# DiltheyLab/HLA-LA

Hardware: AMD Instinct MI355X
Metric: paired reads/sec aligned to PRG graph (higher is better)
Workload: dtype int32

## Files before the change

hla-la_amd/csrc/batch.h:

```cpp
#pragma once
#include "device_common.h"

namespace hlala {

template <template <class> class Ptr> struct DevBatchT {
    int n_pairs, n_reads, n_chains, stride;
    int from_seeds;
    int unpaired;
    Ptr<const int> read_off;
    Ptr<const uint8_t> read_bases;
    Ptr<const uint8_t> read_quals;
    Ptr<const int> chain_off;
    Ptr<const int> read_primary;
    Ptr<const int> chain_read;
    Ptr<const int> chain_contig;
    Ptr<const int> chain_pos;
    Ptr<const int> chain_offset;
    Ptr<const int> chain_as;
    Ptr<const uint8_t> chain_reverse;
    Ptr<const int> cigar_off;
    Ptr<const u32> cigar;
    Ptr<int> seed_status;
    Ptr<int> seed_ncols;
    Ptr<int> seed_begin;
// ... 20 lines not shown
    Ptr<int> ext_edge;
    Ptr<uint8_t> ext_g;
    Ptr<uint8_t> ext_s;
    Ptr<uint8_t> ext_fromseed;
    Ptr<int> ext_firstlast;
    Ptr<int> pair_status;
    Ptr<int> best_chain;
    Ptr<int> n_comb;
    Ptr<double> pair_ll;
    Ptr<double> pair_mapq;
    Ptr<double> mate_mapq;
    Ptr<uint8_t> strands_valid;
    Ptr<uint8_t> sel_mapq;
    Ptr<u64> counters;
    Ptr<int> work_counter;
    Ptr<int> retry_list;
    Ptr<int> pair_multi;
    Ptr<uint8_t> pair_deferred;
    Ptr<int> chain_order;
    Ptr<int> chain_bucket;
    Ptr<int> order_hist;
    int order_shift, order_nb;
    int long_chunk_nodes, long_max_segs;
    int order_cost;
    Ptr<int> chain_row;
    int n_rows;
    Ptr<int> dp_blk;
    Ptr<int> dp_list;
    int dp_nblk;
    int dp_band;
    int dp_band_risky;
    int dp_jf;
    int dp_long;
    Ptr<void> dp_items;
    Ptr<int> dbg;
};
typedef DevBatchT<HostP> DevBatch;
typedef DevBatchT<GlobP> DevBatchG;
static_assert(sizeof(DevBatch) == sizeof(DevBatchG), "one layout");
__device__ __forceinline__ const DevBatchG& dev_view(const DevBatch* p) { return *(const DevBatchG*)p; }
enum { DESC_VALUE = 0, DESC_VIEW = 1, DESC_GENERIC = 2 };
template <int FORM, class D> __device__ __forceinline__ decltype(auto) desc_of(const D& byValue, const D* inMemory)
{
    if constexpr (FORM == DESC_VIEW) return dev_view(inMemory);
    else if constexpr (FORM == DESC_GENERIC) return (*inMemory);
    else return (byValue);
}

template <class BT> __device__ __forceinline__ int ordered_chains(const BT& B) { return B.chain_order ? __builtin_amdgcn_readfirstlane(B.order_hist[B.order_nb - 1]) : B.n_chains; }

template <class BT> __device__ __forceinline__ size_t row_base(const BT& B, int c) { return (size_t)(B.chain_row ? B.chain_row[c] : c) * (size_t)B.stride; }

enum { DPL_BAND16 = 0, DPL_BAND32 = 2, DPL_BAND64 = 4, DPL_JF = 6, DPL_GEN = 10, DPL_N = 14 };
__host__ __device__ inline int dpl_list(int cls, int dir, bool isLong)
{
    if(cls >= 2) return (cls == 2 ? DPL_BAND16 : (cls == 3 ? DPL_BAND32 : DPL_BAND64)) + dir;
    return (cls == 1 ? DPL_JF : DPL_GEN) + 2 * dir + (isLong ? 0 : 1);
}
__host__ __device__ inline int dp_bases_left(int dir, int seqLen, int start_seq) { return dir ? seqLen - start_seq : start_seq; }
__host__ __device__ inline bool dp_is_long(int dpLong, int dir, int seqLen, int start_seq) { return dpLong > 0 && dp_bases_left(dir, seqLen, start_seq) >= dpLong; }
enum { WC_PAIR_MULTI = 40, WC_PAIR_OVER = 72, WC_BAND_FETCH = 48, WC_FO_COUNT = 54, WC_FO_FETCH = 56, WC_BAND_FAILED = 58, WC_BAND_CALLS = 59, WC_JF_FAILED = 60, WC_BAND_WHY = 62, WC_BAND_TIED = 68,
       WC_RETRY_LONG = 88, WC_N = 100 };
__host__ __device__ inline int wc_retry_short(int tier, int dir) { return 12 + 4 * (tier - 1) + 2 * dir; }
__host__ __device__ inline int wc_retry_fetch(int tier, int dir) { return 13 + 4 * (tier - 1) + 2 * dir; }
__host__ __device__ inline int wc_retry_long(int tier, int dir) { return WC_RETRY_LONG + 2 * (tier - 1) + dir; }
__host__ __device__ inline int retry_entry(int w, int nLong, int nChains) { return w < nLong ? w : nChains - 1 - (w - nLong); }
constexpr int BAND_MAXJ16 = 15, BAND_MAXJ32 = 31, BAND_MAXJ64 = 48;

enum {
    CNT_CHAINS_EXT = 0, CNT_DP_CALLS, CNT_DP_ITERS, CNT_DP_CELLS, CNT_SEED_COLS, CNT_OUT_COLS, CNT_EDGES, CNT_ERRORS, CNT_DP_SHARED
};

}
```

hla-la_amd/csrc/hlala_api.hip:

```cpp
#include <cmath>
#include <cstdio>
#include <cstring>
#include <cstdlib>
#include <algorithm>
#include <map>
#include <mutex>
#include <chrono>
#include <thread>
#include <set>
#include <string>
#include <unordered_map>
#include <vector>

#include "../../include/hlala_gpu.h"
#include "batch.h"
#include "flat_graph.hpp"
#include "host_internal.h"

#include "kernel_dp.hip"
#include "kernel_project.hip"
#include "kernel_order.hip"
#include "kernel_pair.hip"
#include "kernel_pair_overflow.hip"
#include "kernel_typer.hip"
// ... 19 lines not shown
    void* p = nullptr; size_t bytes = 0;
};

struct DpClass {
    int grid = 0, block = 0;
    char* slabs = nullptr; size_t slab_bytes = 0;
    const char* name = "";
    void (*launch)(hlala_ctx* c, const DpClass& k, hipStream_t ws, hlala_batch* b, const DpPoolArgs& pool) = nullptr;
};

struct hlala_ctx {
    int device = 0;
    hipStream_t stream = nullptr;
    hipStream_t side = nullptr;
    hipStream_t up = nullptr, rs = nullptr, active = nullptr;
    int tail_pool_k = 1; std::vector<hlala_batch*> tail;
    hipEvent_t evSideTail = nullptr; bool sideTailValid = false;
    hlala_params params{};
    FlatGraph F;
    DevGraph G{};
    DevGraph* dG = nullptr;
    DevTables* dT = nullptr;
    double* d_islog = nullptr;
    long long* d_contig_off = nullptr; uint8_t* d_contig_seq = nullptr; int* d_contig_level = nullptr;
    int n_contigs = 0; std::vector<long long> contig_off;
    std::vector<void*> allocs;
    std::unordered_map<void*, size_t> block_bytes;
    std::multimap<size_t, void*> pool;
    size_t pool_bytes = 0;
    size_t pool_cap = (size_t)176 << 30;
    std::mutex pool_mu;
    std::set<struct hlala_batch*> batches;
    int dp_long_bases = 48;
    int jf_margin = 16;
    int stitch_by_row = 1;
    int stitch_draw = 12;
    bool side_after_pair = false;
    bool rows_all = false;
    bool band_risky = false;
    int band_grid = 0, band_margin = 8;
    DpClass dp[DP_LAST_TIER + 1]; DpClass dp_jf;
    int stitch_grid = 0;
    char* proj_slabs = nullptr; size_t proj_slab_bytes = 0; int proj_grid = 0, pair_grid = 0, pair_lean_grid = 0;
    char* rethread_slabs = nullptr; size_t rethread_slab_bytes = 0; int rethread_grid = 0;
    double* pair_scratch = nullptr;
    char* pair_over_slabs = nullptr; long long pair_over_scratch = 0, pair_over_slab_bytes = 0;
    char* proj_long_slabs = nullptr; size_t proj_long_slab_bytes = 0;
    void* create_scratch = nullptr; size_t create_scratch_bytes = 0; bool create_scratch_pinned = false;
    int long_chunk_nodes = 1 << 20, long_max_segs = 1 << 20;
    int order_cost = 0;
    int order_shift = 8, order_nb = 0;
    int* dbg_host = nullptr;
    int* d_cov = nullptr; int n_cov = 0; int* d_gene_first = nullptr; int* d_gene_last = nullptr; int n_genes = 0;
    struct KeptReads { uint8_t* store = nullptr; long long* start = nullptr; int* length = nullptr; int n = 0; };
    std::vector<KeptReads> kept;
    std::string err;
};

enum BatchEvent {
    EV_PROJECT_BEGIN, EV_PROJECT_END, EV_EXTEND_BEGIN, EV_EXTEND_END, EV_PAIR_BEGIN, EV_PAIR_END,
    EV_DP_BAND_BEGIN, EV_DP_BAND_END,
    EV_DP_BEGIN, EV_DP_CLASS0_END, EV_DP_CLASS2_END, EV_DP_END,
    EV_DP_JUMP_FREE_END,
    EV_DP_CLASS_BEGIN,
    EV_DP_CLASS_END = EV_DP_CLASS_BEGIN + DP_LAST_TIER + 1,
    EV_SIDE_FORK = EV_DP_CLASS_END + DP_LAST_TIER + 1,
// ... 310 lines not shown
        rc = dev_upload(c, c->allocs, lo.data(), lo.size(), (long long**)&G.lp_off); if(rc) return fail(rc);
    }
    UPG(gap_stretch, F.gap_stretch); UPG(lp_seqid, F.lp_seqid); UPG(lp_pos, F.lp_pos);
#undef UPG
    if(contigs && contigs->n_contigs > 0) {
        c->n_contigs = contigs->n_contigs;
        c->contig_off.assign(contigs->contig_off, contigs->contig_off + contigs->n_contigs + 1);
        size_t total = (size_t)c->contig_off.back();
        std::vector<long long> co(c->contig_off.begin(), c->contig_off.end());
        rc = dev_upload(c, c->allocs, co.data(), co.size(), &c->d_contig_off); if(rc) return fail(rc);
        rc = dev_upload(c, c->allocs, contigs->contig_seq, total, &c->d_contig_seq); if(rc) return fail(rc);
        rc = dev_upload(c, c->allocs, contigs->contig_level, total, &c->d_contig_level); if(rc) return fail(rc);
    }
    rc = build_tables(c); if(rc) return fail(rc);
    rc = dev_upload(c, c->allocs, &c->G, 1, &c->dG); if(rc) return fail(rc);
    hipDeviceProp_t prop;
    if(hipGetDeviceProperties(&prop, device) != hipSuccess) { c->err = "hipGetDeviceProperties failed"; return fail(HLALA_E_DEVICE); }
    int cus = prop.multiProcessorCount > 0 ? prop.multiProcessorCount : 256;
    auto slab_pool = [&](char** out, size_t bytes, const char* what) -> int {
        if(device_malloc_retry(c->device, nullptr, (void**)out, bytes) != hipSuccess) { c->err = std::string("hipMalloc(") + what + ") failed"; return HLALA_E_DEVICE; }
        c->allocs.push_back(*out);
        if(hipMemsetAsync(*out, 0, bytes, c->active) != hipSuccess) { c->err = std::string("hipMemset(") + what + ") failed"; return HLALA_E_DEVICE; }
        return 0;
    };
    c->band_grid = cus * 20;
    if(const char* e = getenv("HLALA_DP_BAND")) { if(atoi(e) == 0) c->band_grid = 0; }
    if(const char* e = getenv("HLALA_DP_BAND_RISKY")) c->band_risky = atoi(e) != 0;
    if(const char* e = getenv("HLALA_ROWS_ALL")) c->rows_all = atoi(e) != 0;
    if(const char* e = getenv("HLALA_SIDE_AFTER_PAIR")) c->side_after_pair = atoi(e) != 0;
    if(const char* e = getenv("HLALA_POOL_CAP_GB")) { const long g = atol(e); if(g >= 0 && g <= 1024) c->pool_cap = (size_t)g << 30; }
    if(const char* e = getenv("HLALA_DP_BAND_MARGIN")) { const int m = atoi(e); if(m >= 0 && m <= 24) c->band_margin = m; }
    if(const char* e = getenv("HLALA_DP_JF_MARGIN")) { const int m = atoi(e); if(m >= 0 && m <= 200) c->jf_margin = m; }
    if(const char* e = getenv("HLALA_DP_LONG_BASES")) { const int m = atoi(e); if(m >= 0 && m <= 4096) c->dp_long_bases = m; }
    c->stitch_grid = cus * 20;
    if(const char* e = getenv("HLALA_STITCH_BY_ROW")) c->stitch_by_row = atoi(e) != 0;
    const size_t extBytes = std::max(dp_slab_bytes<DpSmall>(), dp_slab_bytes<DpWide>()), largeBytes = std::max(dp_slab_bytes<DpLarge>(), dp_slab_bytes<DpBroad>());
    DpClass* const dp = c->dp;
    c->dp_jf = dp_class<DpTinyJF, 0>(cus * 4 * DpTinyJF::WAVES, dp_slab_bytes<DpTiny>(), "k_dp<DpTinyJF>");
    dp[0] = dp_class<DpTiny, 0>(cus * 4 * DpTiny::WAVES, dp_slab_bytes<DpTiny>(), "k_dp<DpTiny>");
    dp[1] = dp_class<DpMid, 1>(cus * 16, dp_slab_bytes<DpMid>(), "k_dp<DpMid>");
    dp[2] = dp_class<DpSmall, 2>(cus * 20, extBytes, "k_dp<DpSmall>");
    dp[3] = dp_class<DpWide, 3>(cus * 7, extBytes, "k_dp<DpWide>");
    dp[4] = dp_class<DpBroad, 4>(cus * 3, largeBytes, "k_dp<DpBroad>");
    dp[5] = dp_class<DpLarge, 5>(cus, largeBytes, "k_dp<DpLarge>");
    dp[6] = dp_class<DpHuge, 6>(cus / 4 > 0 ? cus / 4 : 1, dp_inmemory_bytes<DpHuge>(), "k_dp<DpHuge>");
    if((rc = slab_pool(&dp[0].slabs, dp[0].slab_bytes * (size_t)(64 / DpTiny::GW) * (size_t)std::max(dp[0].grid, c->dp_jf.grid), "16-lane DP slabs"))) return fail(rc);
    c->dp_jf.slabs = dp[0].slabs;
    if((rc = slab_pool(&dp[1].slabs, dp[1].slab_bytes * (size_t)(64 / DpMid::GW) * (size_t)dp[1].grid, "32-lane DP slabs"))) return fail(rc);
    if((rc = slab_pool(&dp[2].slabs, extBytes * (size_t)dp[2].grid, "64-lane DP slabs"))) return fail(rc);
    if((rc = slab_pool(&dp[3].slabs, extBytes * (size_t)dp[3].grid, "wide-class DP slabs"))) return fail(rc);
    if((rc = slab_pool(&dp[4].slabs, largeBytes * (size_t)(dp[4].grid + dp[5].grid), "large-class DP slabs"))) return fail(rc);
    dp[5].slabs = dp[4].slabs + largeBytes * (size_t)dp[4].grid;
    if((rc = slab_pool(&dp[6].slabs, dp[6].slab_bytes * (size_t)dp[6].grid, "in-memory DP class"))) return fail(rc);
    c->proj_grid = cus * (c->params.max_columns <= PROJ_CAP_SHORT ? 12 : 8); c->pair_grid = cus * 16; c->pair_lean_grid = cus * 24;
    { int rcp = dev_alloc(c, c->allocs, (size_t)2 * c->pair_grid * PAIR_COMB, &c->pair_scratch, false); if(rcp) return fail(rcp); }
    if(c->params.max_columns > PROJ_CAP) {
        c->proj_grid = cus * 20;
        c->proj_long_slab_bytes = proj_long_slab_bytes();
        c->stitch_draw = 1;
        if(device_malloc_retry(c->device, nullptr, (void**)&c->proj_long_slabs, c->proj_long_slab_bytes * (size_t)c->proj_grid) != hipSuccess) { c->err = "hipMalloc(long-read projection slabs) failed"; return fail(HLALA_E_DEVICE); }
        c->allocs.push_back(c->proj_long_slabs);
    }
    c->proj_slab_bytes = proj_slab_bytes_host(c->params.max_columns, F.max_nodes_per_level);
    if(device_malloc_retry(c->device, nullptr, (void**)&c->proj_slabs, c->proj_slab_bytes * (size_t)c->proj_grid) != hipSuccess) { c->err = "hipMalloc(projection slabs) failed"; return fail(HLALA_E_DEVICE); }
    c->allocs.push_back(c->proj_slabs);
    if(!c->proj_long_slabs) {
// ... 74 lines not shown
}
int hlala_graph_get_gap_stretch(const hlala_ctx* c, uint8_t* in_stretch)
{
    if(!c || !in_stretch) return HLALA_E_ARG;
    memcpy(in_stretch, c->F.gap_stretch.data(), c->F.gap_stretch.size());
    return HLALA_OK;
}


static int batch_alloc_outputs(hlala_ctx* c, hlala_batch* b)
{
    DevBatch& B = b->B;
    size_t nc = (size_t)B.n_chains, nr = (size_t)B.n_reads, np = (size_t)B.n_pairs;
    if(!b->prepared) { B.n_rows = B.n_chains; B.chain_row = nullptr; }
    size_t rowsAlloc = (size_t)(B.n_rows > 0 ? B.n_rows : 1);
    if(b->prepared && nc >= 4096) { const size_t gran = nc / 64; rowsAlloc = (rowsAlloc + gran - 1) / gran * gran; if(rowsAlloc > nc) rowsAlloc = nc; }
    const size_t cs = rowsAlloc * (size_t)B.stride;
    int rc = 0;
#define AL(field, n, zero) do { rc = dev_alloc(c, b->allocs, (n), &B.field, zero); if(rc) return rc; } while(0)
    if(!b->prepared) { AL(seed_status, nc, true); AL(seed_ncols, nc, true); }
    AL(seed_begin, nc, true); AL(seed_end, nc, true); AL(seed_removed, nc, true);
    AL(seed_level, cs, false); AL(seed_edge, cs, false); AL(seed_g, cs, false); AL(seed_s, cs, false);
    AL(ext_status, nc, true); AL(ext_ncols, nc, true); AL(ext_begin, nc, true); AL(ext_end, nc, true); AL(ext_ll, nc, true);
    AL(dp_iters, 2 * nc, true); AL(dp_score, 2 * nc, true); AL(dp_ncols, 2 * nc, true); AL(dp_sb, 2 * nc, true); AL(dp_se, 2 * nc, true); AL(dp_err, 2 * nc, true);
    AL(dp_alias_head, 2 * nc, false); AL(dp_alias_next, 2 * nc, false);
    AL(ext_level, cs, false); AL(ext_edge, cs, false); AL(ext_g, cs, false); AL(ext_s, cs, false); AL(ext_fromseed, cs, false);
    AL(ext_firstlast, 4 * nc, true);
    AL(pair_status, np, true); AL(best_chain, nr, true); AL(n_comb, np, true); AL(pair_ll, np, true); AL(pair_mapq, np, true);
    AL(mate_mapq, nr, true); AL(strands_valid, np, true); AL(sel_mapq, nr * (size_t)B.stride, true);
    AL(pair_deferred, np, true); AL(pair_multi, 7 * np, false); AL(counters, 32, true); AL(work_counter, WC_N, true); AL(retry_list, 16 * nc, false);
    { DpItem* it = nullptr; rc = dev_alloc(c, b->allocs, 2 * nc, &it, false); if(rc) return rc; B.dp_items = it; }
    B.dp_nblk = (int)((nc + 255) / 256); if(B.dp_nblk < 1) B.dp_nblk = 1;
    B.dp_jf = c->jf_margin + 1; B.dp_long = c->dp_long_bases;
    B.dp_band = c->band_grid > 0 ? c->band_margin + 1 : 0;
    B.dp_band_risky = c->band_risky ? 1 : 0;
    AL(dp_blk, (size_t)DPL_N * B.dp_nblk + 1, false); AL(dp_list, 2 * nc, false);
    if(!b->prepared) {
        B.chain_order = nullptr; B.chain_bucket = nullptr; B.order_hist = nullptr; B.order_shift = c->order_shift; B.order_nb = c->order_nb; B.order_cost = c->order_cost; B.long_chunk_nodes = c->long_chunk_nodes; B.long_max_segs = c->long_max_segs;
        if(c->order_nb > 0 && !B.from_seeds && nc > 0) { AL(chain_order, nc, false); AL(chain_bucket, nc, false); AL(order_hist, (size_t)c->order_nb + 1, false); }
    }
    B.dbg = c->dbg_host;
#undef AL
    return 0;
}

static int batch_create_impl(hlala_ctx* c, const hlala_batch_in* in, hlala_batch** out, bool unpaired);
int hlala_batch_create(hlala_ctx* c, const hlala_batch_in* in, hlala_batch** out) { return batch_create_impl(c, in, out, false); }
int hlala_batch_create_unpaired(hlala_ctx* c, const hlala_batch_in* in, hlala_batch** out) { return batch_create_impl(c, in, out, true); }

static int batch_create_impl(hlala_ctx* c, const hlala_batch_in* in, hlala_batch** out, bool unpaired)
{
    DEV_GUARD(c);
    if(!c || !in || !out) return HLALA_E_ARG;
    UploadScope upscope_(c);
    *out = nullptr;
    if(in->n_pairs < 0 || in->n_chains < 0) { c->err = "negative batch sizes"; return HLALA_E_ARG; }
    if(!c->d_contig_off) { c->err = "hlala_batch_create needs contigs (hlala_create was called without them)"; return HLALA_E_STATE; }
    static const bool hostTiming = getenv("HLALA_HOST_TIMING") != nullptr;
    const auto tc0 = std::chrono::steady_clock::now(); auto tc1 = tc0, tc2 = tc0;
    hlala_batch* b = new hlala_batch(); b->ctx = c; c->batches.insert(b);
    DevBatch& B = b->B;
    B.n_pairs = in->n_pairs; B.n_reads = (unpaired ? 1 : 2) * in->n_pairs; B.n_chains = in->n_chains; B.stride = c->params.max_columns; B.from_seeds = 0; B.unpaired = unpaired ? 1 : 0;
    int nr = B.n_reads, nc = B.n_chains;
    auto fail = [&](int rc) { (void)hipStreamSynchronize(c->active); hlala_batch_destroy(b); return rc; };
    const int64_t rb0 = nr > 0 ? in->read_off[0] : 0, cb0 = nr > 0 ? in->chain_off[0] : 0;
    if(nr > 0) {
// ... 279 lines not shown
    return check_launch(c, "k_dp_lists");
}
static int dp_band(hlala_ctx* c, hlala_batch* b)
{
    DevBatch& B = b->B;
    b->band_used = c->band_grid > 0;
    if(!b->band_used) return HLALA_OK;
    const DpItem* items = (const DpItem*)B.dp_items; const u32 seed = c->params.rng_seed + 2u * b->first_chain;
    HIP_TRY(c, hipEventRecord(b->ev[EV_DP_BAND_BEGIN], c->active));
    hipLaunchKernelGGL((k_dp_band<16>), dim3(c->band_grid), dim3(64), 0, c->active, c->G, b->B, items, seed, (const uint8_t*)B.read_bases, c->G.lin_label, c->G.lin_eid);
    hipLaunchKernelGGL((k_dp_band<32>), dim3(c->band_grid), dim3(64), 0, c->active, c->G, b->B, items, seed, (const uint8_t*)B.read_bases, c->G.lin_label, c->G.lin_eid);
    hipLaunchKernelGGL((k_dp_band<64>), dim3(c->band_grid), dim3(64), 0, c->active, c->G, b->B, items, seed, (const uint8_t*)B.read_bases, c->G.lin_label, c->G.lin_eid);
    STEP(check_launch(c, "k_dp_band"));
    HIP_TRY(c, hipEventRecord(b->ev[EV_DP_BAND_END], c->active)); return HLALA_OK;
}
static int dp_classes(hlala_ctx* c, hlala_batch* const* bs, int n, int first, int last, hipStream_t ws)
{
    const DpPoolArgs noPool{};
    DpPoolArgs pool{}; pool.n = n; hlala_batch* b0 = bs[0];
    for(int i = 0; i < n; i++) { const hlala_batch* b = bs[i]; pool.seed[i] = c->params.rng_seed + 2u * b->first_chain; pool.B[i] = b->dB; pool.items[i] = (const DpItem*)b->B.dp_items; pool.bases[i] = (const uint8_t*)b->B.read_bases; }
    for(int tier = first; tier <= last; tier++) {
        const DpClass& k = c->dp[tier];
        if(tier == 0) HIP_TRY(c, hipEventRecord(b0->ev[EV_DP_BEGIN], c->active));
        for(int i = 0; i < n; i++) HIP_TRY(c, hipEventRecord(bs[i]->ev[EV_DP_CLASS_BEGIN + tier], ws));
        if(tier == 0) {
            c->dp_jf.launch(c, c->dp_jf, ws, b0, noPool);
            STEP(check_launch(c, c->dp_jf.name));
            HIP_TRY(c, hipEventRecord(b0->ev[EV_DP_JUMP_FREE_END], ws));
        }
        k.launch(c, k, ws, b0, tier < DP_POOL_TIER ? noPool : pool);
        STEP(check_launch(c, k.name));
        for(int i = 0; i < n; i++) HIP_TRY(c, hipEventRecord(bs[i]->ev[EV_DP_CLASS_END + tier], ws));
        if(tier == 0 || tier == 2) HIP_TRY(c, hipEventRecord(b0->ev[tier == 0 ? EV_DP_CLASS0_END : EV_DP_CLASS2_END], c->active));
    }
    return HLALA_OK;
}
static int side_fork(hlala_ctx* c, hlala_batch* b)
{
    HIP_TRY(c, hipEventRecord(b->ev[EV_SIDE_FORK], c->active)); HIP_TRY(c, hipStreamWaitEvent(c->side, b->ev[EV_SIDE_FORK], 0));
    HIP_TRY(c, hipEventRecord(b->ev[EV_SIDE_BEGIN], c->side)); b->side_used = true;
    return HLALA_OK;
}
static int side_mark(hlala_ctx* c, hlala_batch* b)
{
    HIP_TRY(c, hipEventRecord(b->ev[EV_DONE], c->side)); b->side_inflight = true;
    HIP_TRY(c, hipEventRecord(c->evSideTail, c->side)); c->sideTailValid = true;
    return HLALA_OK;
}
static int stitch_main(hlala_ctx* c, hlala_batch* b, int mode)
{
    const int sgrid = b->B.n_chains < c->stitch_grid ? b->B.n_chains : c->stitch_grid;
    hipLaunchKernelGGL(k_stitch_chains, dim3(sgrid), dim3(64), 0, c->active, c->G, c->dT, b->B, (const uint8_t*)b->B.pair_deferred, mode, c->stitch_draw, c->stitch_by_row);
    return check_launch(c, "k_stitch_chains");
}
static int stitch_side(hlala_ctx* c, hlala_batch* b)
{
    const int pgrid = (b->B.n_pairs + 63) / 64, cap = c->stitch_grid / 20;
    hipLaunchKernelGGL(k_stitch_chains, dim3(pgrid < cap ? (pgrid > 0 ? pgrid : 1) : cap), dim3(64), 0, c->side, c->G, c->dT, b->B, (const uint8_t*)b->B.pair_deferred, 2, 0, 0);
    return check_launch(c, "k_stitch_chains (side)");
}
static int extend_end(hlala_ctx* c, hlala_batch* b) { HIP_TRY(c, hipEventRecord(b->ev[EV_EXTEND_END], c->active)); b->staged |= 2; return mark_main(c, b); }
static int pair_begin(hlala_ctx* c, hlala_batch* b) { HIP_TRY(c, hipMemsetAsync(b->B.work_counter + 2, 0, sizeof(int), c->active)); HIP_TRY(c, hipEventRecord(b->ev[EV_PAIR_BEGIN], c->active)); return HLALA_OK; }
static int pair_pass(hlala_ctx* c, hlala_batch* b, hipStream_t st, int mode)
{
    DevBatch& B = b->B;
    const int grid = B.n_pairs < c->pair_grid ? B.n_pairs : c->pair_grid, lean = B.n_pairs < c->pair_lean_grid ? B.n_pairs : c->pair_lean_grid;
// ... 570 lines not shown
    for(int i = 0; i < n; i++) { hlala_ctx* c = m->ctxs[(size_t)i]; DevGuard g(c->device);
        if(!c->d_cov) { c->n_cov = (int)nl; int rc = dev_alloc(c, c->allocs, nl, &c->d_cov, true); if(rc) { m->err = c->err; return rc; } }
        if(hipStreamSynchronize(c->rs) != hipSuccess || hipStreamSynchronize(c->stream) != hipSuccess) { m->err = "hlala_reduce_coverage: a context's stream failed"; return HLALA_E_DEVICE; } }
    ncclResult_t r = g_rccl.GroupStart();
    for(int i = 0; i < n && r == ncclSuccess; i++) r = g_rccl.Reduce(m->ctxs[(size_t)i]->d_cov, i == 0 ? (void*)m->covAcc : nullptr, nl, ncclInt32, ncclSum, 0, m->comms[(size_t)i], m->streams[(size_t)i]);
    const ncclResult_t re = g_rccl.GroupEnd();
    if(r == ncclSuccess) r = re;
    if(r != ncclSuccess) { m->err = std::string("RCCL reduce: ") + g_rccl.GetErrorString(r); return HLALA_E_DEVICE; }
    for(int i = 0; i < n; i++) { hlala_ctx* c = m->ctxs[(size_t)i]; DevGuard g(c->device);
        if(hipStreamSynchronize(m->streams[(size_t)i]) != hipSuccess) { m->err = "RCCL reduce: stream failed"; return HLALA_E_DEVICE; }
        if(reset && hipMemset(c->d_cov, 0, nl * sizeof(int)) != hipSuccess) { m->err = "hipMemset failed"; return HLALA_E_DEVICE; } }
    DevGuard g0(c0->device);
    if(hipMemcpy(bases_per_level, m->covAcc, nl * sizeof(int), hipMemcpyDeviceToHost) != hipSuccess) { m->err = "coverage: copy to the host failed"; return HLALA_E_DEVICE; }
    return HLALA_OK;
}


int hlala_batch_get_stats(hlala_ctx* c, hlala_batch* b, hlala_batch_stats* out)
{
    DEV_GUARD(c);
    ReaderScope rscope_(c, b); if(rscope_.rc) return rscope_.rc;
    if(!c || !b || !out) return HLALA_E_ARG;
    memset(out, 0, sizeof(*out));
    if(!b->outputs_ready) return HLALA_OK;
    HIP_TRY(c, hipStreamSynchronize(c->active));
    u64 cnt[16];
    HIP_TRY(c, hipMemcpyAsync(cnt, b->B.counters, sizeof(cnt), hipMemcpyDeviceToHost, c->active)); HIP_TRY(c, hipStreamSynchronize(c->active));
    if((b->staged & 1) && !b->B.from_seeds) (void)hipEventElapsedTime(&out->ms_project, b->ev[EV_PROJECT_BEGIN], b->ev[EV_PROJECT_END]);
    if(b->staged & 2) { (void)hipEventElapsedTime(&out->ms_extend, b->ev[EV_EXTEND_BEGIN], b->ev[EV_EXTEND_END]); if(b->B.n_chains > 0) { (void)hipEventElapsedTime(&out->ms_extend_retry, b->ev[EV_DP_CLASS0_END], b->ev[b->side_used ? EV_DP_CLASS2_END : EV_DP_END]); (void)hipEventElapsedTime(&out->ms_dp_main, b->ev[EV_DP_BEGIN], b->ev[EV_DP_CLASS0_END]);
          for(int k = 0; k <= DP_LAST_TIER; k++) (void)hipEventElapsedTime(&out->ms_dp_class[k], b->ev[EV_DP_CLASS_BEGIN + k], b->ev[EV_DP_CLASS_END + k]);
          (void)hipEventElapsedTime(&out->ms_dp_jump_free, b->ev[EV_DP_CLASS_BEGIN], b->ev[EV_DP_JUMP_FREE_END]);
          if(b->band_used) (void)hipEventElapsedTime(&out->ms_dp_band, b->ev[EV_DP_BAND_BEGIN], b->ev[EV_DP_BAND_END]);
          if(b->side_used) (void)hipEventElapsedTime(&out->ms_side, b->ev[EV_SIDE_BEGIN], b->ev[EV_SIDE_END]); } }
    { int wc[WC_N]; HIP_TRY(c, hipMemcpyAsync(wc, b->B.work_counter, sizeof(wc), hipMemcpyDeviceToHost, c->active)); HIP_TRY(c, hipStreamSynchronize(c->active)); out->n_chains_retried = 0; for(int k = 1; k <= 6; k++) out->n_dp_class[k] = wc[wc_retry_short(k, 0)] + wc[wc_retry_short(k, 1)] + wc[wc_retry_long(k, 0)] + wc[wc_retry_long(k, 1)];
      for(int k = 1; k <= 6; k++) out->n_chains_retried += out->n_dp_class[k]; out->n_dp_retried_large = out->n_dp_class[5];
      out->n_dp_band = b->band_used ? wc[WC_BAND_CALLS] : 0; out->n_dp_band_failed = b->band_used ? wc[WC_BAND_FAILED] : 0; out->n_dp_jump_free_failed = wc[WC_JF_FAILED];
      out->n_dp_class[0] = wc[8] + wc[9] - out->n_dp_band + out->n_dp_band_failed; out->n_dp_jump_free = wc[6]; }
    if(b->staged & 4) (void)hipEventElapsedTime(&out->ms_pair, b->ev[EV_PAIR_BEGIN], b->ev[EV_PAIR_END]);
    out->n_chains_extended = (int64_t)cnt[CNT_CHAINS_EXT]; out->n_dp_calls = (int64_t)cnt[CNT_DP_CALLS];
    out->n_dp_iterations = (int64_t)cnt[CNT_DP_ITERS]; out->n_dp_cells = (int64_t)cnt[CNT_DP_CELLS];
    out->n_seed_columns = (int64_t)cnt[CNT_SEED_COLS]; out->n_out_columns = (int64_t)cnt[CNT_OUT_COLS];
    out->n_edges_touched = (int64_t)cnt[CNT_EDGES]; out->n_errors = (int64_t)cnt[CNT_ERRORS]; out->n_dp_shared = (int64_t)cnt[CNT_DP_SHARED];
    return HLALA_OK;
}

}

static int typer_tables(hlala_ctx* c, std::vector<void*>& tmp, TyperTables** out)
{
    TyperTables T;
    double insertionP = c->params.long_read_mode ? 0.075 : 0.001, deletionP = insertionP;
    T.ll_ins_actual = log(insertionP) + log(1.0 / 4.0);
    T.ll_deletion = log(deletionP);
    T.ll_match_mismatch = log(1 - insertionP - deletionP);
    for(int q = 0; q < 256; q++) {
        double pCorrect = host_PhredToPCorrect((unsigned char)(q < 33 ? 33 : q));
        if(pCorrect > 0.999) pCorrect = 0.999;
        if(pCorrect == 0) pCorrect = 0.001;
        T.ll_match[q] = log(pCorrect);
        double pIncorrect = (1 - pCorrect) * (1.0 / 3.0);
        T.ll_mismatch[q] = log(pIncorrect);
    }
    return dev_upload(c, tmp, &T, 1, out);
}

static void hand_over(std::vector<void*>& from, std::vector<void*>* to, void* p)
{
// ... 1320 lines not shown
```

hla-la_amd/csrc/kernel_dp.hip:

```cpp
#include "batch.h"
#include "../../include/hlala_gpu.h"

namespace hlala {

enum { K_DIAG = 0, K_GGAP = 1, K_SGAP = 2, K_HOP = 3, K_JUMP = 4 };
enum { M_D = 0, M_GG = 1, M_SG = 2 };
enum { PH_IDLE = 0, PH_RUN, PH_SELECT, PH_BT, PH_EXPAND, PH_DONE };

constexpr u64 HKEY_EMPTY = ~0ull;
#ifndef HLALA_DP_PROFILE_LOG2
#define HLALA_DP_PROFILE_LOG2 18
#endif
#ifndef HLALA_EARLY_GEN_MAX
#define HLALA_EARLY_GEN_MAX 0xFFFFFE
#endif
constexpr int DP_EARLY_GEN_MAX = HLALA_EARLY_GEN_MAX;
constexpr int EXT_PENDING = 0x7FFFFFFF;
constexpr int DP_BT_STEPS_PER_TRIP = 32;

#ifndef HLALA_DP_TAIL_THREADS
#define HLALA_DP_TAIL_THREADS 128
#endif
constexpr int DP_TAIL_THREADS = HLALA_DP_TAIL_THREADS;
#ifndef HLALA_DP_TINY_WAVES
// ... 1350 lines not shown
__global__ void k_dp_lists(const DevBatch B, const DpItem* __restrict__ items)
{
    const int t = blockIdx.x * blockDim.x + threadIdx.x;
    const int nOrd = ordered_chains(B);
    int kL = -1, kR = -1;
    if(t < nOrd) {
        const int4* sl = (const int4*)(items + t); const int4* sr = (const int4*)(items + (size_t)B.n_chains + t);
        const int4 a = sl[0], b = sr[0];
        if(a.x >= 0) kL = dpl_list(sl[1].z, 0, dp_is_long(B.dp_long, 0, a.z, a.w));
        if(b.x >= 0) kR = dpl_list(sr[1].z, 1, dp_is_long(B.dp_long, 1, b.z, b.w));
    }
    __shared__ int waveCnt[DPL_N][4];
    const int lane = lane_id(), wv = (int)(threadIdx.x >> 6);
    u64 m[DPL_N];
#pragma unroll
    for(int k = 0; k < DPL_N; k++) m[k] = __ballot(kL == k || kR == k);
    if(lane == 0) {
#pragma unroll
        for(int k = 0; k < DPL_N; k++) waveCnt[k][wv] = (int)__popcll(m[k]);
    }
    __syncthreads();
    const u64 below = (1ull << lane) - 1ull;
#pragma unroll
    for(int k = 0; k < DPL_N; k++) {
        if(kL == k || kR == k) {
            int before = 0;
            for(int w2 = 0; w2 < wv; w2++) before += waveCnt[k][w2];
            const int pos = B.dp_blk[(size_t)k * gridDim.x + blockIdx.x] + before + (int)__popcll(m[k] & below);
            B.dp_list[pos] = kR == k ? B.n_chains + t : t;
        }
    }
}

struct DpPoolArgs {
    int n;
    u32 seed[DP_POOL_MAX];
    const DevBatch* B[DP_POOL_MAX];
    const DpItem* items[DP_POOL_MAX];
    const uint8_t* bases[DP_POOL_MAX];
};

template <class C, int TIER, class DG, class DB>
__device__ __forceinline__ void dp_class_run(const DG& G, const DB& B, const DpItem* __restrict__ items, DpLdsT<C>& S, DpSlabT<C> sl, u64* sortScratch, const u32 rng_seed,
                                             const int4* __restrict__ nrecOut, const int4* __restrict__ nrecIn, const uint8_t* __restrict__ readBases);

template <class C, int TIER> __host__ __device__ constexpr int dp_desc_form() { return ((TIER == 0 && C::JF) || TIER == 3 || TIER == 5) ? DESC_VIEW : DESC_GENERIC; }

template <class C, int TIER>
__global__ __launch_bounds__(C::THREADS, C::WAVES) void k_dp(const DevGraph* __restrict__ Gp, const DevBatch* __restrict__ Bp, const DpItem* __restrict__ items,
                                                        char* slabs, size_t slabBytes, u32 rng_seed,
                                                        const int4* __restrict__ nrecOut, const int4* __restrict__ nrecIn, const uint8_t* __restrict__ readBasesArg, const DpPoolArgs pool)
{
    constexpr int GW = C::GW;
    constexpr int NG = GW >= 64 ? 1 : 64 / GW;
    static_assert(C::THREADS == (GW >= 64 ? GW : 64), "block size");
    constexpr int FORM = dp_desc_form<C, TIER>();
    const auto& G = desc_of<FORM>(*Gp, Gp);
    const int g = (int)((threadIdx.x & 63) / GW);
    DpLdsT<C>* Sp; DpSlabT<C> sl; u64* sortScratch = nullptr;
    if constexpr (C::IN_MEMORY) {
        __shared__ u64 scratch[2 * DP_SORT_SCRATCH];
        char* base = slabs + (size_t)blockIdx.x * slabBytes;
        Sp = (DpLdsT<C>*)base; sl.base = base + ((sizeof(DpLdsT<C>) + 255) & ~(size_t)255); sortScratch = scratch;
    } else {
        __shared__ DpLdsT<C> SS[NG];
        Sp = &SS[g]; sl.base = slabs + ((size_t)blockIdx.x * NG + g) * slabBytes;
// ... 346 lines not shown
```

hla-la_amd/csrc/kernel_dp_band.hip:

```cpp
#include "batch.h"

namespace hlala {

constexpr int BAND_ABSENT = -20000;
constexpr int BAND_DRAW = 16;
constexpr int BAND_TIES = 16;

template <int GW_> struct BandCfg;
template <> struct BandCfg<16> { static constexpr int GW = 16, MAXJ = BAND_MAXJ16, REACH = 64, MAXD = 96, WAVES = 5; };
template <> struct BandCfg<32> { static constexpr int GW = 32, MAXJ = BAND_MAXJ32, REACH = 96, MAXD = 128, WAVES = 5; };
template <> struct BandCfg<64> { static constexpr int GW = 64, MAXJ = BAND_MAXJ64, REACH = 112, MAXD = 160, WAVES = 5; };

template <class C>
struct __align__(16) BandLds {
    u32 bt[C::MAXD / 8][C::GW];
    unsigned short steps[C::MAXD];
    unsigned short tieD[BAND_TIES];
    u32 ls[C::REACH];
};

template <int GW> __device__ __forceinline__ int band_prev(int v, int gl)
{
    if(GW == 16) return dpp_mov<0x111>(DP_NEG, v);
    int r = __builtin_amdgcn_update_dpp(DP_NEG, v, 0x138, 0xF, 0xF, false);
// ... 214 lines not shown
            if(nx < 0) live = false; else item = nx;
            first = false;
            BAND_T(3);
        }
        if(has && fail && gl == 0) {
            const int q = atomicAdd(&B.work_counter[WC_FO_COUNT + dirPass], 1);
            B.retry_list[(size_t)(14 + dirPass) * (size_t)B.n_chains + q] = idx;
            atomicAdd(&B.work_counter[WC_BAND_FAILED], 1); atomicAdd(&B.work_counter[WC_BAND_WHY + fail], 1);
        }
        WSYNC();
#ifdef HLALA_BAND_TIMING
        tAcc[4] += 0; if(lane == 0) atomicAdd(&B.counters[22], 1ull);
#endif
    }
#ifdef HLALA_BAND_TIMING
    if(lane == 0 && GW == 16) { for(int i = 0; i < 5; i++) atomicAdd(&B.counters[16 + i], (u64)tAcc[i]); atomicAdd(&B.counters[21], (u64)tAcc[5]); }
#endif
}

template <int GW>
__global__ __launch_bounds__(64, BandCfg<GW>::WAVES) void k_dp_band(const DevGraph G, const DevBatch B, const DpItem* __restrict__ items, const u32 rng_seed,
                                                                    const uint8_t* __restrict__ readBases, const u32* __restrict__ linLabel, const int* __restrict__ linEid)
{
    typedef BandCfg<GW> C;
    __shared__ BandLds<C> SS[64 / GW];
    BandLds<C>& S = SS[lane_id() / GW];
    u64 accCalls = 0, accIters = 0, accCells = 0, accEdges = 0;
    band_pass<C, false>(G, B, items, rng_seed, readBases, linLabel, linEid, S, accCalls, accIters, accCells, accEdges);
    band_pass<C, true>(G, B, items, rng_seed, readBases, linLabel, linEid, S, accCalls, accIters, accCells, accEdges);
    if((lane_id() & (GW - 1)) == 0 && accCalls) {
        atomicAdd(&B.counters[CNT_DP_CALLS], accCalls); atomicAdd(&B.counters[CNT_DP_ITERS], accIters);
        atomicAdd(&B.counters[CNT_DP_CELLS], accCells); atomicAdd(&B.counters[CNT_EDGES], accEdges);
    }
}

}
```

Measured before the change: 5.740 million.

## Sort DP retry lists by remaining bases using counting sort before next tier

Adds two kernels that build a histogram of remaining-bases keys for each retry list and then scatter-reorder the list in descending cost order. They run after the first two DP retry tiers, so the next tier processes work of similar length together and the long items start first. This is meant to reduce load imbalance and divergence in the retry DP. In exchange it adds two extra kernel launches and a scratch copy per tier, and it enlarges the work-counter array. It also adds an optional band-kernel timing probe behind a compile flag.

```diff
diff --git a/hla-la_amd/csrc/batch.h b/hla-la_amd/csrc/batch.h
--- a/hla-la_amd/csrc/batch.h
+++ b/hla-la_amd/csrc/batch.h
@@ -76,6 +76,7 @@
     int dp_band_risky;
     int dp_jf;
     int dp_long;
+    int retry_block;
     Ptr<void> dp_items;
     Ptr<int> dbg;
 };
@@ -104,7 +105,9 @@
 __host__ __device__ inline int dp_bases_left(int dir, int seqLen, int start_seq) { return dir ? seqLen - start_seq : start_seq; }
 __host__ __device__ inline bool dp_is_long(int dpLong, int dir, int seqLen, int start_seq) { return dpLong > 0 && dp_bases_left(dir, seqLen, start_seq) >= dpLong; }
 enum { WC_PAIR_MULTI = 40, WC_PAIR_OVER = 72, WC_BAND_FETCH = 48, WC_FO_COUNT = 54, WC_FO_FETCH = 56, WC_BAND_FAILED = 58, WC_BAND_CALLS = 59, WC_JF_FAILED = 60, WC_BAND_WHY = 62, WC_BAND_TIED = 68,
-       WC_RETRY_LONG = 88, WC_N = 100 };
+       WC_RETRY_LONG = 88, WC_RETRY_HIST = 100, RETRY_NB = 32, RETRY_ORDER_TIERS = 2, WC_N = WC_RETRY_HIST + RETRY_ORDER_TIERS * 4 * 2 * RETRY_NB };
+__host__ __device__ inline int wc_retry_hist(int tier, int part, int cursor) { return WC_RETRY_HIST + (((tier - 1) * 4 + part) * 2 + cursor) * RETRY_NB; }
+__host__ __device__ inline int retry_key(int basesLeft) { const int k = basesLeft >> 3; return k < 0 ? 0 : (k < RETRY_NB ? k : RETRY_NB - 1); }
 __host__ __device__ inline int wc_retry_short(int tier, int dir) { return 12 + 4 * (tier - 1) + 2 * dir; }
 __host__ __device__ inline int wc_retry_fetch(int tier, int dir) { return 13 + 4 * (tier - 1) + 2 * dir; }
 __host__ __device__ inline int wc_retry_long(int tier, int dir) { return WC_RETRY_LONG + 2 * (tier - 1) + dir; }
diff --git a/hla-la_amd/csrc/hlala_api.hip b/hla-la_amd/csrc/hlala_api.hip
--- a/hla-la_amd/csrc/hlala_api.hip
+++ b/hla-la_amd/csrc/hlala_api.hip
@@ -75,6 +75,8 @@
     std::mutex pool_mu;
     std::set<struct hlala_batch*> batches;
     int dp_long_bases = 48;
+    int dp_cost_order = 1;
+    int retry_block = 256;
     int jf_margin = 16;
     int stitch_by_row = 1;
     int stitch_draw = 12;
@@ -451,6 +453,8 @@
     if(const char* e = getenv("HLALA_DP_BAND_MARGIN")) { const int m = atoi(e); if(m >= 0 && m <= 24) c->band_margin = m; }
     if(const char* e = getenv("HLALA_DP_JF_MARGIN")) { const int m = atoi(e); if(m >= 0 && m <= 200) c->jf_margin = m; }
     if(const char* e = getenv("HLALA_DP_LONG_BASES")) { const int m = atoi(e); if(m >= 0 && m <= 4096) c->dp_long_bases = m; }
+    if(const char* e = getenv("HLALA_DP_COST_ORDER")) c->dp_cost_order = atoi(e) != 0;
+    if(const char* e = getenv("HLALA_RETRY_BLOCK")) { const int m = atoi(e); if(m >= 1 && m <= RETRY_ORDER_THREADS) c->retry_block = m; }
     c->stitch_grid = cus * 20;
     if(const char* e = getenv("HLALA_STITCH_BY_ROW")) c->stitch_by_row = atoi(e) != 0;
     const size_t extBytes = std::max(dp_slab_bytes<DpSmall>(), dp_slab_bytes<DpWide>()), largeBytes = std::max(dp_slab_bytes<DpLarge>(), dp_slab_bytes<DpBroad>());
@@ -591,6 +595,7 @@
     { DpItem* it = nullptr; rc = dev_alloc(c, b->allocs, 2 * nc, &it, false); if(rc) return rc; B.dp_items = it; }
     B.dp_nblk = (int)((nc + 255) / 256); if(B.dp_nblk < 1) B.dp_nblk = 1;
     B.dp_jf = c->jf_margin + 1; B.dp_long = c->dp_long_bases;
+    B.retry_block = c->retry_block;
     B.dp_band = c->band_grid > 0 ? c->band_margin + 1 : 0;
     B.dp_band_risky = c->band_risky ? 1 : 0;
     AL(dp_blk, (size_t)DPL_N * B.dp_nblk + 1, false); AL(dp_list, 2 * nc, false);
@@ -936,6 +941,12 @@
         STEP(check_launch(c, k.name));
         for(int i = 0; i < n; i++) HIP_TRY(c, hipEventRecord(bs[i]->ev[EV_DP_CLASS_END + tier], ws));
         if(tier == 0 || tier == 2) HIP_TRY(c, hipEventRecord(b0->ev[tier == 0 ? EV_DP_CLASS0_END : EV_DP_CLASS2_END], c->active));
+        if(tier < RETRY_ORDER_TIERS && c->dp_cost_order) {
+            const dim3 grid(RETRY_ORDER_BLOCKS, 4);
+            hipLaunchKernelGGL(k_retry_hist, grid, dim3(RETRY_ORDER_THREADS), 0, ws, b0->B, (const DpItem*)b0->B.dp_items, tier + 1);
+            hipLaunchKernelGGL(k_retry_order, grid, dim3(RETRY_ORDER_THREADS), 0, ws, b0->B, (const DpItem*)b0->B.dp_items, tier + 1);
+            STEP(check_launch(c, "k_retry_order"));
+        }
     }
     return HLALA_OK;
 }
@@ -1572,7 +1583,7 @@
           (void)hipEventElapsedTime(&out->ms_dp_jump_free, b->ev[EV_DP_CLASS_BEGIN], b->ev[EV_DP_JUMP_FREE_END]);
           if(b->band_used) (void)hipEventElapsedTime(&out->ms_dp_band, b->ev[EV_DP_BAND_BEGIN], b->ev[EV_DP_BAND_END]);
           if(b->side_used) (void)hipEventElapsedTime(&out->ms_side, b->ev[EV_SIDE_BEGIN], b->ev[EV_SIDE_END]); } }
-    { int wc[WC_N]; HIP_TRY(c, hipMemcpyAsync(wc, b->B.work_counter, sizeof(wc), hipMemcpyDeviceToHost, c->active)); HIP_TRY(c, hipStreamSynchronize(c->active)); out->n_chains_retried = 0; for(int k = 1; k <= 6; k++) out->n_dp_class[k] = wc[wc_retry_short(k, 0)] + wc[wc_retry_short(k, 1)] + wc[wc_retry_long(k, 0)] + wc[wc_retry_long(k, 1)];
+    { int wc[WC_RETRY_HIST]; HIP_TRY(c, hipMemcpyAsync(wc, b->B.work_counter, sizeof(wc), hipMemcpyDeviceToHost, c->active)); HIP_TRY(c, hipStreamSynchronize(c->active)); out->n_chains_retried = 0; for(int k = 1; k <= 6; k++) out->n_dp_class[k] = wc[wc_retry_short(k, 0)] + wc[wc_retry_short(k, 1)] + wc[wc_retry_long(k, 0)] + wc[wc_retry_long(k, 1)];
       for(int k = 1; k <= 6; k++) out->n_chains_retried += out->n_dp_class[k]; out->n_dp_retried_large = out->n_dp_class[5];
       out->n_dp_band = b->band_used ? wc[WC_BAND_CALLS] : 0; out->n_dp_band_failed = b->band_used ? wc[WC_BAND_FAILED] : 0; out->n_dp_jump_free_failed = wc[WC_JF_FAILED];
       out->n_dp_class[0] = wc[8] + wc[9] - out->n_dp_band + out->n_dp_band_failed; out->n_dp_jump_free = wc[6]; }
diff --git a/hla-la_amd/csrc/kernel_dp.hip b/hla-la_amd/csrc/kernel_dp.hip
--- a/hla-la_amd/csrc/kernel_dp.hip
+++ b/hla-la_amd/csrc/kernel_dp.hip
@@ -1406,6 +1406,63 @@
     }
 }
 
+constexpr int RETRY_ORDER_THREADS = 256, RETRY_ORDER_BLOCKS = 64;
+__device__ __forceinline__ size_t retry_part_place(bool isShort, int j, int nChains) { return isShort ? (size_t)(nChains - 1 - j) : (size_t)j; }
+__device__ __forceinline__ int retry_item_key(const DpItem* __restrict__ items, int idx, int dir)
+{
+    const int4 a = *(const int4*)(items + idx);
+    return retry_key(dp_bases_left(dir, a.z, a.w));
+}
+
+__global__ __launch_bounds__(RETRY_ORDER_THREADS) void k_retry_hist(const DevBatch B, const DpItem* __restrict__ items, const int tier)
+{
+    __shared__ int cnt[RETRY_NB];
+    const int part = blockIdx.y, dir = part >> 1; const bool isShort = part & 1;
+    const int n = B.work_counter[isShort ? wc_retry_short(tier, dir) : wc_retry_long(tier, dir)];
+    const int per = B.retry_block;
+    if(n < 2 || (int)blockIdx.x * per >= n) return;
+    int* row = B.retry_list + (size_t)(2 * (tier - 1) + dir) * (size_t)B.n_chains; int* scratch = B.retry_list + (size_t)(12 + dir) * (size_t)B.n_chains;
+    if(threadIdx.x < RETRY_NB) cnt[threadIdx.x] = 0;
+    __syncthreads();
+    for(int j0 = blockIdx.x * per; j0 < n; j0 += gridDim.x * per) {
+        const int j = j0 + (int)threadIdx.x;
+        if((int)threadIdx.x < per && j < n) {
+            const size_t at = retry_part_place(isShort, j, B.n_chains);
+            const int idx = row[at]; scratch[at] = idx;
+            atomicAdd(&cnt[retry_item_key(items, idx, dir)], 1);
+        }
+    }
+    __syncthreads();
+    if(threadIdx.x < RETRY_NB && cnt[threadIdx.x]) atomicAdd(&B.work_counter[wc_retry_hist(tier, part, 0) + threadIdx.x], cnt[threadIdx.x]);
+}
+
+__global__ __launch_bounds__(RETRY_ORDER_THREADS) void k_retry_order(const DevBatch B, const DpItem* __restrict__ items, const int tier)
+{
+    __shared__ int first[RETRY_NB], cnt[RETRY_NB], base[RETRY_NB];
+    const int part = blockIdx.y, dir = part >> 1; const bool isShort = part & 1;
+    const int n = B.work_counter[isShort ? wc_retry_short(tier, dir) : wc_retry_long(tier, dir)];
+    const int per = B.retry_block;
+    if(n < 2 || (int)blockIdx.x * per >= n) return;
+    int* row = B.retry_list + (size_t)(2 * (tier - 1) + dir) * (size_t)B.n_chains; const int* scratch = B.retry_list + (size_t)(12 + dir) * (size_t)B.n_chains;
+    int* cursor = B.work_counter + wc_retry_hist(tier, part, 1);
+    if(threadIdx.x < RETRY_NB) {
+        const int* hist = B.work_counter + wc_retry_hist(tier, part, 0);
+        int before = 0; for(int k = RETRY_NB - 1; k > (int)threadIdx.x; k--) before += hist[k];
+        first[threadIdx.x] = before;
+    }
+    for(int j0 = blockIdx.x * per; j0 < n; j0 += gridDim.x * per) {
+        if(threadIdx.x < RETRY_NB) cnt[threadIdx.x] = 0;
+        __syncthreads();
+        const int j = j0 + (int)threadIdx.x; const bool has = (int)threadIdx.x < per && j < n;
+        int idx = 0, key = 0, rank = 0;
+        if(has) { idx = scratch[retry_part_place(isShort, j, B.n_chains)]; key = retry_item_key(items, idx, dir); rank = atomicAdd(&cnt[key], 1); }
+        __syncthreads();
+        if(threadIdx.x < RETRY_NB && cnt[threadIdx.x]) base[threadIdx.x] = atomicAdd(&cursor[threadIdx.x], cnt[threadIdx.x]);
+        __syncthreads();
+        if(has) row[retry_part_place(isShort, first[key] + base[key] + rank, B.n_chains)] = idx;
+    }
+}
+
 struct DpPoolArgs {
     int n;
     u32 seed[DP_POOL_MAX];
diff --git a/hla-la_amd/csrc/kernel_dp_band.hip b/hla-la_amd/csrc/kernel_dp_band.hip
--- a/hla-la_amd/csrc/kernel_dp_band.hip
+++ b/hla-la_amd/csrc/kernel_dp_band.hip
@@ -270,6 +270,13 @@
         atomicAdd(&B.counters[CNT_DP_CALLS], accCalls); atomicAdd(&B.counters[CNT_DP_ITERS], accIters);
         atomicAdd(&B.counters[CNT_DP_CELLS], accCells); atomicAdd(&B.counters[CNT_EDGES], accEdges);
     }
-}
-
-}
+#if defined(HLALA_DP_TIMING) && HLALA_DP_TIMING + 0 == 2
+    if(lane_id() == 0) {
+        constexpr int KI = GW == 16 ? 5 : (GW == 32 ? 6 : 7);
+        const u64 now = (u64)wall_clock64();
+        atomicMax((unsigned long long*)&B.counters[16 + 2 * KI], (unsigned long long)~now); atomicMax((unsigned long long*)&B.counters[17 + 2 * KI], (unsigned long long)now);
+    }
+#endif
+}
+
+}
```

Result: no change. 5.733 million (median of 2 runs) (-0.1%).
